# Yoshiki172/Deep-Learning-based-RGBA-Image-Compression-with-Masked-Window-based-Attention

Measured on NVIDIA B200. Metric: 768x512 RGBA images/s (AutoEncoderRGB_Journal encode + decode forward); masked-attn kernel % of roofline, higher is better.
Workload: dtype f32 (attention: fp16 hi+lo split operands, 3 tcgen05 passes, f32 accumulate = f32-faithful; 4x4 attention plain f32; GDN contraction bf16x3 split + f32 accumulate; convolutions fp16 hi+lo split operands, 3 tcgen05 passes, chunked f32 accumulation outside the tensor core = f32-faithful)

## Files before the change

deep-learning-based-rgba-image-compression-with-masked-window-based-attention_b200/_abi.py:

```python
from __future__ import annotations

import ctypes
import os
from ctypes import c_char_p, c_float, c_int, c_int32, c_int64, c_void_p, POINTER

import torch

_PKG_DIR = os.path.dirname(os.path.abspath(__file__))
LIB_PATH = os.path.join(_PKG_DIR, "libmwa_b200.so")

MWA_OK = 0
ALGO_AUTO, ALGO_SIMT, ALGO_TCGEN05 = 0, 1, 2
ABI_VERSION = 1

_SIGNATURES = {
    "mwa_b200_abi_version": (c_int, []),
    "mwa_b200_status_string": (c_char_p, [c_int]),
    "mwa_b200_last_cuda_error": (c_char_p, []),
    "gdn_param_bytes": (c_int64, [c_int]),
    "gdn_prepare": (c_int, [c_void_p, c_void_p, c_int, c_float, c_float, c_float, c_void_p, c_int64, c_void_p]),
    "gdn_forward": (c_int, [c_void_p, c_void_p, c_void_p, c_int64, c_int, c_int64, c_int, c_int, c_int, c_void_p]),
    "gdn_forward_planes": (c_int, [c_void_p, c_void_p, c_void_p, c_int, c_int, c_void_p, c_int64, c_int, c_int, c_int, c_int,
                                   c_void_p]),
    "gdn_backward_workspace_bytes": (c_int64, [c_int64, c_int, c_int64]),
# ... 3 lines not shown
    "gdn_bwd_square": (c_int, [c_void_p, c_void_p, c_int64, c_void_p]),
    "gdn_bwd_dn": (c_int, [c_void_p, c_void_p, c_void_p, c_void_p, c_void_p, c_int64, c_int, c_int64, c_int, c_int,
                           c_void_p]),
    "gdn_bwd_dx": (c_int, [c_void_p, c_void_p, c_void_p, c_void_p, c_int64, c_void_p]),
    "gdn_bwd_finalize": (c_int, [c_void_p, c_void_p, c_void_p, c_void_p, c_float, c_float, c_void_p, c_void_p,
                                 c_void_p, c_int64, c_int, c_int64, c_int, c_void_p]),
    "mwa_param_bytes": (c_int64, [c_int, c_int, c_int]),
    "mwa_prepare": (c_int, [c_void_p, c_void_p, c_void_p, c_void_p, c_void_p, c_int, c_int, c_int, c_float,
                            c_void_p, c_int64, c_void_p]),
    "mwa_debug_set_timing_buffer": (None, [c_void_p]),
    "mwa_workspace_bytes": (c_int64, [c_int, c_int, c_int, c_int]),
    "mwa_fast_path_needs_nchw": (c_int, [c_int, c_int, c_int]),
    "conv_image_bytes": (c_int64, [c_int, c_int, c_int, c_int, c_int]),
    "conv_split_bytes": (c_int64, [c_int, c_int, c_int, c_int]),
    "conv_prepare": (c_int, [c_void_p, c_int, c_int, c_int, c_int, c_int, c_void_p, c_int64, c_void_p]),
    "conv_forward": (c_int, [c_void_p, c_int64, c_void_p, c_void_p, c_void_p, c_int64, c_void_p, c_void_p, c_void_p, c_int,
                             c_int, c_int, c_int, c_int, c_int, c_int, c_int, c_int, c_void_p]),
    "gemm_tokens_forward": (c_int, [c_void_p, c_int64, c_int, c_void_p, c_void_p, c_int, c_void_p, c_void_p, c_void_p, c_void_p,
                                    c_void_p]),
    "conv_act_split": (c_int, [c_void_p, c_int64, c_int, c_int, c_int, c_int, c_int, c_void_p, c_void_p, c_int, c_int, c_void_p]),
    "conv_forward_ex": (c_int, [c_void_p, c_int64, c_void_p, c_void_p, c_int, c_void_p, c_void_p, c_void_p, c_int64,
                                c_void_p, c_int64, c_void_p, c_int64, c_void_p, c_void_p, c_int, c_int, c_int, c_void_p,
                                c_int, c_int, c_int, c_int, c_int, c_int, c_int, c_int, c_int, c_void_p, c_void_p]),
    "mwa_forward": (c_int, [c_void_p, c_void_p, c_void_p, c_void_p, c_int, c_int, c_int, c_int, c_int, c_int, c_int,
                            c_int, c_int, c_void_p, c_void_p, c_int64, c_void_p]),
    "window_attention_forward": (c_int, [c_void_p, c_void_p, c_void_p, c_void_p, c_int64, c_int, c_int, c_int, c_int,
                                         c_void_p]),
    "mwa_backward": (c_int, [c_void_p] * 12 + [c_int] * 8 + [c_void_p]),
    "window_attention_backward": (c_int, [c_void_p] * 10 + [c_int64, c_int, c_int, c_int, c_int, c_void_p]),
    "mwa_bwd_gather": (c_int, [c_void_p] * 6 + [c_int] * 7 + [c_void_p]),
    "mwa_bwd_core": (c_int, [c_void_p] * 8 + [c_int64] + [c_int] * 7 + [c_void_p]),
    "mwa_bwd_scatter": (c_int, [c_void_p] * 3 + [c_int] * 7 + [c_void_p]),
    "gate_residual_forward": (c_int, [c_void_p, c_void_p, c_void_p, c_void_p, c_int64, c_void_p]),
    "gate_residual_backward": (c_int, [c_void_p, c_void_p, c_void_p, c_void_p, c_void_p, c_int64, c_void_p]),
    "round_ste_forward": (c_int, [c_void_p, c_void_p, c_int64, c_int64, c_int64, c_int64, c_void_p]),
    "quantize_offset_forward": (c_int, [c_void_p, c_void_p, c_void_p, c_int64, c_int64, c_int64, c_int64, c_int64,
                                        c_int, c_int64, c_void_p]),
    "lrp_add_forward": (c_int, [c_void_p, c_void_p, c_void_p, c_int64, c_int64, c_int64, c_int64, c_int64, c_void_p]),
    "quantize_levels_forward": (c_int, [c_void_p, c_void_p, c_int64, c_float, c_void_p]),
    "alpha_pyramid_level_offset": (c_int64, [c_int, c_int, c_int, c_int]),
    "alpha_pyramid_forward": (c_int, [c_void_p, c_void_p, c_void_p, c_int, c_int, c_int, c_int, c_int, c_void_p]),
    "ms_ssim_level_forward": (c_int, [c_void_p, c_void_p, c_void_p, c_int, c_int, c_int, c_int, c_float, c_void_p, c_void_p,
                                      c_void_p]),
    "ms_ssim_pool_forward": (c_int, [c_void_p, c_void_p, c_void_p, c_int, c_int, c_int, c_int, c_void_p, c_void_p, c_void_p,
                                     c_void_p]),
    "rans_encode_with_indexes": (c_int64, [c_void_p, c_void_p, c_int64, c_void_p, c_int, c_void_p, c_void_p, c_int, c_void_p,
# ... 94 lines not shown
```

deep-learning-based-rgba-image-compression-with-masked-window-based-attention_b200/codec.py:

```python
from __future__ import annotations

import math

import numpy as np
import torch
import torch.nn as nn
import torch.nn.functional as F

from . import quant
from .layers.GDN import GDN
from .layers.Masked_Attention import Win_noShift_Attention, conv3x3
from .layers.conv import ACT_ADD2, ACT_LRP, ACT_QUANT, ACT_RELU, Conv2d, ConvStack, ConvTranspose2d, SplitAct
from .layers.SupplyMask import SupplyMaskToTransform, alpha_pyramid


def _conv(cin, cout, k, stride=1):
    return Conv2d(cin, cout, k, stride=stride, padding=k // 2)


def _deconv5(cin, cout):
    return ConvTranspose2d(cin, cout, 5, stride=2, padding=2, output_padding=1)


def _subpel(cin, cout, r=2):
    return nn.Sequential(Conv2d(cin, cout * r * r, 3, padding=1), nn.PixelShuffle(r))


class EnhancementBlock(nn.Module):

    def __init__(self, n=32):
        super().__init__()
        self.conv1 = Conv2d(n, n, 3, padding=1)
        self.relu = nn.ReLU(inplace=True)
        self.conv2 = Conv2d(n, n, 3, padding=1)

    def forward(self, x, **kw):
        if self.conv1.input_ps(x) is None:
            return self.conv2(self.conv1(x, act=ACT_RELU), residual=x)
        return self.conv2(self.conv1(x, act=ACT_RELU, emit_ps=1, want_dense=False),
                          residual=x.dense if isinstance(x, SplitAct) else x, **kw)


class DSE(nn.Module):

    def __init__(self, n=32):
        super().__init__()
        self.input_conv = Conv2d(3, n, 1)
        self.enh1, self.enh2, self.enh3 = EnhancementBlock(n), EnhancementBlock(n), EnhancementBlock(n)
        self.output_conv = Conv2d(n, 3, 1)

    def forward(self, x):
        if self.input_conv.input_ps(x) is None:
            first = self.input_conv(x)
            t = self.enh3(self.enh2(self.enh1(first)))
            return self.output_conv(t + first, residual=x)
        first = self.input_conv(x, emit_ps=1)
        t = self.enh2(self.enh1(first, emit_ps=1), emit_ps=1)
        h = self.enh3.conv1(t, act=ACT_RELU, emit_ps=1, want_dense=False)
        s = self.enh3.conv2(h, act=ACT_ADD2, residual=t.dense, aux=first.dense, emit_ps=1, want_dense=False)
        return self.output_conv(s, residual=x)


def _gdn_into(gdn, x, consumer):
    ps = consumer.input_ps(x) if torch.is_tensor(x) and x.dim() == 4 and x.shape[1] == consumer.in_channels else None
    return gdn.request_planes(ps)(x) if ps else gdn(x)


def _attention_into(attention, x, mask, consumer):
    ps = consumer.input_ps(x) if torch.is_tensor(x) and x.dim() == 4 and x.shape[1] == consumer.in_channels else None
    if ps and attention.conv_a[0].conv[0].input_ps(x) is not None:
        return attention.request_planes(ps)(x, mask)
    return attention(x, mask)


class Analysis_transform(nn.Module):

    def __init__(self, N=192, M=320):
        super().__init__()
        self.x1 = _conv(3, N, 5, 2)
        self.gdn1 = GDN(N)
        self.x2 = _conv(N, N, 5, 2)
        self.gdn2 = GDN(N)
        self.attention1 = Win_noShift_Attention(dim=N, num_heads=8, window_size=8, shift_size=4)
        self.x3 = _conv(N, N, 5, 2)
        self.gdn3 = GDN(N)
        self.x4 = Conv2d(N, M, 1)
        self.attention2 = Win_noShift_Attention(dim=M, num_heads=8, window_size=4, shift_size=2)

    def forward(self, input, mask, me1, me2, me3, me4):
        y = _gdn_into(self.gdn1, self.x1(input), self.x2)
        y = self.gdn2(self.x2(y))
        y = _attention_into(self.attention1, y, me2, self.x3)
        y = _gdn_into(self.gdn3, self.x3(y), self.x4)
        return self.attention2(self.x4(y), me3)


class Synthesis_transform(nn.Module):

    def __init__(self, N=196, M=320):
        super().__init__()
        self.attention1 = Win_noShift_Attention(dim=M, num_heads=8, window_size=4, shift_size=2)
        self.x1 = Conv2d(M, N, 1)
        self.igdn1 = GDN(N, inverse=True)
        self.x2 = _deconv5(N, N)
        self.igdn2 = GDN(N, inverse=True)
        self.attention2 = Win_noShift_Attention(N, num_heads=8, window_size=8, shift_size=4)
        self.x3 = _deconv5(N, N)
        self.igdn3 = GDN(N, inverse=True)
        self.x4 = _deconv5(N, 3)
        self.dse = DSE(32)

    def forward(self, input, reconmask, md1, md2, md3, md4):
        y = _attention_into(self.attention1, input, md3, self.x1)
        y = _gdn_into(self.igdn1, self.x1(y), self.x2)
        y = self.igdn2(self.x2(y))
        y = _attention_into(self.attention2, y, md2, self.x3)
        y = _gdn_into(self.igdn3, self.x3(y), self.x4)
        return self.dse(self.x4(y))


class EntropyBottleneck(nn.Module):

    def __init__(self, channels, filters=(3, 3, 3, 3), init_scale=10.0):
        super().__init__()
        self.channels = channels
        f = (1,) + tuple(filters) + (1,)
        scale = init_scale ** (1.0 / (len(filters) + 1))
        for i in range(len(filters) + 1):
            init = math.log(math.expm1(1.0 / scale / f[i + 1]))
            self.register_parameter(f"_matrix{i:d}", nn.Parameter(torch.full((channels, f[i + 1], f[i]), init)))
            self.register_parameter(f"_bias{i:d}", nn.Parameter(torch.rand(channels, f[i + 1], 1) - 0.5))
            if i < len(filters):
                self.register_parameter(f"_factor{i:d}", nn.Parameter(torch.zeros(channels, f[i + 1], 1)))
        self.nlayers = len(filters) + 1
        self.quantiles = nn.Parameter(torch.tensor([-init_scale, 0.0, init_scale]).repeat(channels, 1, 1))

    def _get_medians(self):
        return self.quantiles[:, :, 1:2].detach().reshape(1, -1, 1, 1)

    def _logits_cumulative(self, v):
        for i in range(self.nlayers):
# ... 364 lines not shown
```

deep-learning-based-rgba-image-compression-with-masked-window-based-attention_b200/csrc/conv_tc.cu:

```cuda
#include <cstring>
#include <cuda.h>
#include "common.cuh"
#include "params.cuh"
#include "status.cuh"

namespace b200 {
namespace {

__host__ __device__ constexpr int conv_colparts(int nbmax) { return nbmax <= 64 ? 2 : 4; }
__host__ __device__ constexpr int conv_threads(int nbmax) { return (3 + 4 * conv_colparts(nbmax)) * 32; }
constexpr int kMaxTaps = 25, kMaxClasses = 4, kMaxGroups = 4;
constexpr int kTileH = 16, kTileW = 8;
enum { kActNone = 0, kActGelu = 1, kActRelu = 2, kActQuant = 3, kActLrp = 4, kActGate = 5, kActAdd2 = 6 };

struct ConvIo {
    const float* bias;
    const float* residual;
    float* out;
    int64_t out_bs;
    const float* aux;
    int64_t aux_bs;
    float* out2;
    int64_t out2_bs;
    uint16_t* sp_hi;
    uint16_t* sp_lo;
    int sp_ps, sp_cstride, sp_coff, sp_cvalid;
    const float* in_scale;
    int out_cl;
};

struct ConvTap {
    int16_t row;
    int16_t slab;
};
struct ConvGroup {
    int8_t plane, ntaps;
    int16_t first;
};
struct ConvPlan {
    int B, Cin, Cout, Npad, nblocks, nb;
    int KB;
    int GH, GW;
    int Ho, Wo, os;
    int ncls;
    int ntaps[kMaxClasses], ngroups[kMaxClasses];
    int8_t qy[kMaxClasses], qx[kMaxClasses];
    ConvGroup groups[kMaxClasses][kMaxGroups];
    ConvTap taps[kMaxClasses][kMaxTaps];
    int th, tw, tw_log2;
    int hy, hx, oy0, ox0;
    int a_half;
    int act;
    int merged;
    int nslabs;
    int sa, sb;
    int bparts;
    int resident;
    int dual;
    int nbuf_log2, bstride;
    int ncat;
    int b_region;
    int chunk;
    int nchunks[kMaxClasses];
    int tiles_y, tiles_x;
};

__device__ __forceinline__ uint64_t umma_desc_k_sw128_sbo(uint32_t smem_addr, uint32_t sbo_bytes) {
    uint64_t d = 0;
    d |= static_cast<uint64_t>((smem_addr & 0x3FFFFu) >> 4);
    d |= static_cast<uint64_t>(1) << 16;
    d |= static_cast<uint64_t>(sbo_bytes >> 4) << 32;
    d |= static_cast<uint64_t>(1) << 46;
    d |= static_cast<uint64_t>(2) << 61;
    return d;
}

__device__ __forceinline__ void tma_load_5d(void* dst_smem, const void* map, int c0, int c1, int c2, int c3, int c4, uint64_t* bar) {
    asm volatile(
        "cp.async.bulk.tensor.5d.shared::cluster.global.tile.mbarrier::complete_tx::bytes [%0], [%1, {%2,%3,%4,%5,%6}], [%7];" ::"r"(
            smem_u32(dst_smem)),
        "l"(map), "r"(c0), "r"(c1), "r"(c2), "r"(c3), "r"(c4), "r"(smem_u32(bar))
        : "memory");
}

__device__ __forceinline__ uint16_t conv_f16_bits(float v) { return __half_as_ushort(__float2half_rn(v)); }

__global__ void __launch_bounds__(256)
// ... 220 lines not shown
        } else {
            y[u] = v + rv[u];
        }
        if (!FULL && u >= nvalid) y[u] = 0.f;
    }
    if (dst != nullptr) {
#pragma unroll
        for (int u = 0; u < 8; ++u)
            if (FULL || u < nvalid) dst[u * ohw] = y[u];
    }
    if (sph != nullptr) {
        uint32_t hi[4], lo[4];
#pragma unroll
        for (int u = 0; u < 4; ++u) {
            hi[u] = pack_f16x2(y[2 * u], y[2 * u + 1]);
            const float2 hf = __half22float2(*reinterpret_cast<const __half2*>(&hi[u]));
            lo[u] = pack_f16x2(y[2 * u] - hf.x, y[2 * u + 1] - hf.y);
        }
        *reinterpret_cast<uint4*>(sph) = make_uint4(hi[0], hi[1], hi[2], hi[3]);
        *reinterpret_cast<uint4*>(spl) = make_uint4(lo[0], lo[1], lo[2], lo[3]);
    }
}

template <int NBMAX, bool kCL = false, bool kSingle = false>
__global__ void __launch_bounds__(conv_threads(NBMAX), 1)
conv_tc_kernel(const __grid_constant__ CUtensorMap map_hi, const __grid_constant__ CUtensorMap map_lo,
               const uint8_t* __restrict__ image, const float* __restrict__ inv_scale, const __grid_constant__ ConvIo io,
               const __grid_constant__ ConvPlan P) {
    extern __shared__ __align__(1024) uint8_t smem[];
    __shared__ uint64_t bars[2 * 4 + 2 * 8 + 2 * 4];
    __shared__ uint32_t tmem_slot;
    __shared__ uint2 s_tap[kMaxClasses * kMaxTaps + 1];
    const uint32_t sb = smem_u32(smem);
    const int warp = threadIdx.x >> 5, lane = threadIdx.x & 31;
    const int SA = P.sa, SB = P.sb;
    uint64_t* a_full = bars;
    uint64_t* a_empty = bars + 4;
    uint64_t* b_full = bars + 8;
    uint64_t* b_empty = bars + 16;
    uint64_t* part_full = bars + 24;
    uint64_t* part_empty = bars + 28;
    const uint32_t nbl = uint32_t(P.nbuf_log2), nbm = (1u << nbl) - 1u, bstride = uint32_t(P.bstride);
    const uint32_t b_bytes = uint32_t(P.nb) * 128u;
    const uint32_t b_entry = P.bparts == 2 ? b_bytes : 2u * b_bytes;
    const uint32_t a_slot = 2u * uint32_t(P.a_half);
    const uint32_t b_base = uint32_t(SA) * a_slot;
    if (threadIdx.x == 0) {
        if (sb & 1023u) __trap();
        for (int i = 0; i < SA; ++i) {
            mbar_init(a_full + i, 1);
            mbar_init(a_empty + i, 1);
        }
        for (int i = 0; i < SB; ++i) {
            mbar_init(b_full + i, 1);
            mbar_init(b_empty + i, 1);
        }
        for (int i = 0; i < 4; ++i) {
            mbar_init(part_full + i, 1);
            mbar_init(part_empty + i, 4 * conv_colparts(NBMAX) * 32);
        }
        fence_mbar_init();
    }
    if (warp == 1) tmem_alloc<512>(&tmem_slot);
    float* s_scale = reinterpret_cast<float*>(smem + b_base + P.b_region);
    float* s_bias = s_scale + P.Npad;
    for (int i = threadIdx.x; i < P.Npad; i += conv_threads(NBMAX)) {
        s_scale[i] = inv_scale[i] * (io.in_scale ? 1.f / __ldg(io.in_scale) : 1.f);
        const int co = P.merged ? (i & 7) : i;
        s_bias[i] = (io.bias != nullptr && co < P.Cout) ? io.bias[co] : 0.f;
    }
    for (int i = threadIdx.x; i < kMaxClasses * kMaxTaps; i += conv_threads(NBMAX)) {
        const ConvTap tp = P.taps[i / kMaxTaps][i % kMaxTaps];
        s_tap[i] = make_uint2(uint32_t(tp.row) * 8u, uint32_t(tp.slab * P.KB * 2) * ((uint32_t(P.nb) * 128u) >> 4));
    }
    tc_fence_before_sync();
    __syncthreads();
    tc_fence_after_sync();
    const uint32_t tm = tmem_slot;

    const int tiles_img = P.tiles_y * P.tiles_x;
    const int ntiles = P.B * tiles_img * P.ncls * P.nblocks;
    struct TileIt {
        int nblk, tx, ty, cls, b;
        int d_nblk, d_tx, d_ty, d_cls, d_b;
        __device__ __forceinline__ void init(int t, int step, const ConvPlan& P) {
            auto split = [&](int v, int& nb_, int& tx_, int& ty_, int& cl_, int& b_) {
                nb_ = v % P.nblocks; v /= P.nblocks;
                tx_ = v % P.tiles_x; v /= P.tiles_x;
                ty_ = v % P.tiles_y; v /= P.tiles_y;
                cl_ = v % P.ncls;
                b_ = v / P.ncls;
            };
// ... 275 lines not shown
                                    for (int j = 0; j < 8; ++j) acc[c0 + 8 + j] += __uint_as_float(v1[j]);
                                }
                            }
                        }
                    }
                    if (ch < nchunks - 1) {
                        tc_fence_before_sync();
                        mbar_arrive(part_empty + buf);
                    } else {
#pragma unroll
                        for (int c0 = 0; c0 < NBQ; c0 += 8) {
                            if (c0 < ncols) {
                                uint32_t v[8];
#pragma unroll
                                for (int j = 0; j < 8; ++j) v[j] = __float_as_uint(acc[c0 + j]);
                                tmem_st_x8(tm + lane_addr + buf * bstride + col0 + c0, v);
                            }
                        }
                        tmem_wait_st();
                    }
                }
            }
            if (nchunks == 1) ++c;
            float* dst = io.out ? (kCL ? io.out + pix * io.out_bs + cbase : io.out + b * io.out_bs + cbase * ohw + pix) : nullptr;
            float* dst2 = io.out2 ? io.out2 + b * io.out2_bs + cbase * ohw + pix : nullptr;
            int64_t spo = 0;
            if (io.sp_hi != nullptr) {
                const int sh = io.sp_ps - 1;
                const int hp = P.Ho >> sh, wp = P.Wo >> sh;
                const int plane = ((oy & sh) << sh) + (ox & sh);
                spo = (((int64_t(b) << (2 * sh)) + plane) * hp + (oy >> sh)) * wp + (ox >> sh);
                spo = spo * io.sp_cstride + io.sp_coff + cbase;
            }
            const int act = P.act;
            const int64_t estride = kCL ? 1 : ohw;
#pragma unroll 1
            for (int j0 = 0; j0 < ncols; j0 += 8) {
                uint32_t tv[8];
                tmem_ld_x8(tm + lane_addr + buf * bstride + col0 + j0, tv);
                if (NBMAX <= 64 && P.ncat && nchunks == 1) {
                    uint32_t t2[8];
                    tmem_ld_x8(tm + lane_addr + buf * bstride + P.nb + col0 + j0, t2);
                    tmem_wait_ld();
#pragma unroll
                    for (int u = 0; u < 8; ++u) tv[u] = __float_as_uint(__uint_as_float(tv[u]) + __uint_as_float(t2[u]));
                }
// ... 175 lines not shown
    P.bparts = P.nb > 96 ? 2 : 1;
    if (P.nblocks == 1 && image <= budget) {
        P.resident = 1; P.bparts = 1; P.sb = 1; P.b_region = int(image);
    } else {
        const int entry = P.nb * 128 * (P.bparts == 2 ? 1 : 2);
        P.sb = budget / entry;
        if (P.sb > 8) P.sb = 8;
        if (P.sb < 2) return MWA_ERR_UNSUPPORTED;
        P.b_region = P.sb * entry;
    }
    P.dual = P.resident && P.ncls == 1 && P.ngroups[0] == 1 && P.KB == 1 && P.nchunks[0] == 1 && P.ntaps[0] > 1;
    P.ncat = P.nb <= 64 ? 1 : 0;
    P.nbuf_log2 = (P.nb <= 128 && !P.dual) ? 2 : 1;
    P.bstride = P.nbuf_log2 == 2 ? 128 : 256;
    if (P.dual) {
        const int room = 224 * 1024 - 2 * P.Npad * 4 - P.b_region;
        P.sa = room / (2 * P.a_half);
        if (P.sa > 4) P.sa = 4;
        if (P.sa < 2) P.sa = 2;
    }
    return MWA_OK;
}

int conv_smem_bytes(const ConvPlan& P) { return P.sa * 2 * P.a_half + P.b_region + 2 * P.Npad * 4 + 1024; }

}
}

using namespace b200;

extern "C" {

int64_t conv_image_bytes(int kind, int Cin, int Cout, int k, int stride) {
    ConvPlan P;
    if (Cin <= 0 || Cout <= 0 || build_plan(P, kind, 1, Cin, Cout, 16, 16, k, stride, 0) != MWA_OK) return MWA_ERR_UNSUPPORTED;
    return int64_t(P.nslabs) * P.KB * 2 * P.Npad * 128 + int64_t(P.Npad) * 4;
}

int64_t conv_split_bytes(int B, int Cin, int H, int W) {
    const int64_t Cpad = (Cin + 7) / 8 * 8;
    return int64_t(B) * H * W * Cpad * 2;
}

int conv_prepare(const float* w, int kind, int Cin, int Cout, int k, int stride, void* image, int64_t image_bytes, void* stream) {
    if (!w || !image) return MWA_ERR_INVALID;
    const int wflip = kind == 2;
    if (wflip) {
// ... 10 lines not shown
    float* inv_scale = reinterpret_cast<float*>(img + int64_t(P.nslabs) * P.KB * 2 * P.Npad * 128);
    const int wmode = P.merged ? 3 : wflip ? 2 : kind;
    conv_prepare_kernel<<<P.Npad, 256, 0, static_cast<cudaStream_t>(stream)>>>(w, Cin, Cout, k, wmode, P.Npad, P.KB, P.nslabs,
                                                                              inv_scale, img);
    return check_launch("conv_prepare");
}

int conv_act_split(const float* x, int64_t x_batch_stride, int B, int C, int H, int W, int ps, void* out_hi, void* out_lo,
                   int out_cstride, int out_coff, void* stream) {
    if (!x || !out_hi || !out_lo || B < 0 || C <= 0 || H <= 0 || W <= 0 || (ps != 1 && ps != 2)) return MWA_ERR_INVALID;
    const int Cpad = (C + 7) / 8 * 8;
    if (out_cstride % 8 != 0 || out_coff % 8 != 0 || out_coff < 0 || out_coff + Cpad > out_cstride || H % ps || W % ps)
        return MWA_ERR_INVALID;
    if (!aligned16(out_hi) || !aligned16(out_lo)) return MWA_ERR_ALIGNMENT;
    if (B == 0) return MWA_OK;
    return launch_act_split(x, x_batch_stride, B, C, out_cstride, H, W, ps, static_cast<uint16_t*>(out_hi) + out_coff,
                            static_cast<uint16_t*>(out_lo) + out_coff, static_cast<cudaStream_t>(stream));
}

static int conv_forward_impl(const float* x, int64_t x_batch_stride, void* in_hi, void* in_lo, int in_cstride,
                    const float* bias, const float* residual, float* out, int64_t out_batch_stride, const float* aux,
                    int64_t aux_batch_stride, float* out2, int64_t out2_batch_stride, void* out_hi, void* out_lo,
                    int out_ps, int out_cstride, int out_coff, const void* image, int kind, int B, int Cin, int Cout, int H,
                    int W, int k, int stride, int act, const float* in_scale, void* stream, int out_cl) {
    if (!image || !in_hi || !in_lo || (!out && !out_hi)) return MWA_ERR_INVALID;
    if (B < 0 || Cin <= 0 || Cout <= 0 || H <= 0 || W <= 0 || act < 0 || act > kActAdd2) return MWA_ERR_INVALID;
    if (act >= kActQuant && !aux) return MWA_ERR_INVALID;
    if ((out_hi != nullptr) != (out_lo != nullptr)) return MWA_ERR_INVALID;
    if (B == 0) return MWA_OK;
    ConvPlan P;
    int rc = build_plan(P, kind, B, Cin, Cout, H, W, k, stride, act);
    if (rc != MWA_OK) return rc;
    if (!aligned16(in_hi) || !aligned16(in_lo) || !aligned16(image)) return MWA_ERR_ALIGNMENT;
    if (P.merged && (out_hi != nullptr || act >= kActQuant)) return MWA_ERR_UNSUPPORTED;
    if (int64_t(B) * Cout * P.Ho * P.Wo >= (int64_t(1) << 31)) return MWA_ERR_UNSUPPORTED;
    cudaStream_t st = static_cast<cudaStream_t>(stream);
    const int ps = (kind == 0 && stride == 2) ? 2 : 1;
    int cstride = in_cstride;
    if (x != nullptr) {
        cstride = (Cin + 7) / 8 * 8;
        rc = launch_act_split(x, x_batch_stride, B, Cin, cstride, H, W, ps, static_cast<uint16_t*>(in_hi),
                              static_cast<uint16_t*>(in_lo), st, in_scale);
        if (rc != MWA_OK) return rc;
    } else if (cstride < Cin || cstride % 8 != 0) {
        return MWA_ERR_INVALID;
    }
    ConvIo io;
    memset(&io, 0, sizeof(io));
    io.bias = bias; io.residual = residual; io.out = out; io.out_bs = out_batch_stride;
    io.aux = aux; io.aux_bs = aux_batch_stride; io.out2 = out2; io.out2_bs = out2_batch_stride;
    io.in_scale = in_scale;
    io.out_cl = out_cl;
    if (out_hi != nullptr) {
        if (!aligned16(out_hi) || !aligned16(out_lo)) return MWA_ERR_ALIGNMENT;
        if ((out_ps != 1 && out_ps != 2) || out_cstride % 8 != 0 || out_coff % 8 != 0 || out_coff < 0 ||
            out_coff + (Cout + 7) / 8 * 8 > out_cstride || P.Ho % out_ps != 0 || P.Wo % out_ps != 0)
            return MWA_ERR_INVALID;
        io.sp_hi = static_cast<uint16_t*>(out_hi); io.sp_lo = static_cast<uint16_t*>(out_lo);
        io.sp_ps = out_ps; io.sp_cstride = out_cstride; io.sp_coff = out_coff; io.sp_cvalid = (Cout + 7) / 8 * 8;
    }
    CUtensorMap mh, ml;
    memset(&mh, 0, sizeof(mh));
    memset(&ml, 0, sizeof(ml));
    rc = conv_plane_map(in_hi, B, ps * ps, H / ps, W / ps, Cin, cstride, P.hx, P.hy, &mh);
    if (rc != MWA_OK) return rc;
    rc = conv_plane_map(in_lo, B, ps * ps, H / ps, W / ps, Cin, cstride, P.hx, P.hy, &ml);
    if (rc != MWA_OK) return rc;
    const int smem = conv_smem_bytes(P);
    const int ntiles = B * P.tiles_y * P.tiles_x * P.ncls * P.nblocks;
    const int grid = ntiles < kNumSMs ? ntiles : kNumSMs;
    const uint8_t* img = static_cast<const uint8_t*>(image);
    const float* inv_scale = reinterpret_cast<const float*>(img + int64_t(P.nslabs) * P.KB * 2 * P.Npad * 128);
#define CONV_LAUNCH_K(NB, SINGLE)                                                                                              \
    do {                                                                                                                       \
        MWA_TRY_CUDA(cudaFuncSetAttribute(conv_tc_kernel<NB, false, SINGLE>, cudaFuncAttributeMaxDynamicSharedMemorySize, smem), \
                     "conv_forward(attr)");                                                                                    \
        conv_tc_kernel<NB, false, SINGLE><<<grid, conv_threads(NB), smem, st>>>(mh, ml, img, inv_scale, io, P);                \
    } while (0)
#define CONV_LAUNCH(NB)                                                                                                        \
    do {                                                                                                                       \
        if (NB >= 128 && single) CONV_LAUNCH_K(NB, (NB >= 128));                                                               \
        else CONV_LAUNCH_K(NB, false);                                                                                         \
    } while (0)
    bool single = true;
    for (int c = 0; c < P.ncls; ++c) single = single && P.nchunks[c] == 1;
    if (out_cl) {
        MWA_TRY_CUDA(cudaFuncSetAttribute(conv_tc_kernel<192, true>, cudaFuncAttributeMaxDynamicSharedMemorySize, smem),
                     "gemm_tokens_forward(attr)");
        conv_tc_kernel<192, true><<<grid, conv_threads(192), smem, st>>>(mh, ml, img, inv_scale, io, P);
        return check_launch("gemm_tokens_forward");
    }
    if (P.nb <= 32) CONV_LAUNCH(32);
    else if (P.nb <= 64) CONV_LAUNCH(64);
    else if (P.nb <= 128) CONV_LAUNCH(128);
    else CONV_LAUNCH(192);
#undef CONV_LAUNCH
#undef CONV_LAUNCH_K
    return check_launch("conv_forward");
}

int conv_forward_ex(const float* x, int64_t x_batch_stride, void* in_hi, void* in_lo, int in_cstride,
                    const float* bias, const float* residual, float* out, int64_t out_batch_stride, const float* aux,
                    int64_t aux_batch_stride, float* out2, int64_t out2_batch_stride, void* out_hi, void* out_lo,
                    int out_ps, int out_cstride, int out_coff, const void* image, int kind, int B, int Cin, int Cout, int H,
                    int W, int k, int stride, int act, const float* in_scale, void* stream) {
    return conv_forward_impl(x, x_batch_stride, in_hi, in_lo, in_cstride, bias, residual, out, out_batch_stride, aux,
                             aux_batch_stride, out2, out2_batch_stride, out_hi, out_lo, out_ps, out_cstride, out_coff, image,
                             kind, B, Cin, Cout, H, W, k, stride, act, in_scale, stream, 0);
}

int gemm_tokens_forward(const float* x, int64_t T, int Cin, const float* bias, float* out, int Cout, const void* image,
                        void* split_hi, void* split_lo, const float* in_scale, void* stream) {
    if (!x || !out || !image || !split_hi || !split_lo || T < 0 || Cin <= 0 || Cout <= 0) return MWA_ERR_INVALID;
    if (T == 0) return MWA_OK;
    if (T % 32 != 0 || Cout % 8 != 0 || T / 32 > 2000000) return MWA_ERR_UNSUPPORTED;
    if (!aligned16(x) || !aligned16(out) || !aligned16(split_hi) || !aligned16(split_lo)) return MWA_ERR_ALIGNMENT;
    const int cstride = (Cin + 7) / 8 * 8;
    cudaStream_t st = static_cast<cudaStream_t>(stream);
    const int64_t items = T * ((Cin + 7) / 8);
    int64_t blocks = (items + 255) / 256;
    if (blocks > kNumSMs * 16) blocks = kNumSMs * 16;
    conv_split_cl_kernel<<<unsigned(blocks), 256, 0, st>>>(x, T, Cin, cstride, static_cast<uint16_t*>(split_hi),
                                                          static_cast<uint16_t*>(split_lo), in_scale);
    int rc = check_launch("gemm_tokens_forward(split)");
    if (rc != MWA_OK) return rc;
    return conv_forward_impl(nullptr, 0, split_hi, split_lo, cstride, bias, nullptr, out, Cout, nullptr, 0, nullptr, 0, nullptr,
                             nullptr, 0, 0, 0, image, 0, 1, Cin, Cout, int(T / 32), 32, 1, 1, kActNone, in_scale, stream, 1);
}

int conv_forward(const float* x, int64_t x_batch_stride, const float* bias, const float* residual, float* out,
                 int64_t out_batch_stride, const void* image, void* split_hi, void* split_lo, int kind, int B, int Cin,
// ... 8 lines not shown
```

deep-learning-based-rgba-image-compression-with-masked-window-based-attention_b200/layers/conv.py:

```python
from __future__ import annotations

import torch
import torch.nn as nn
import torch.nn.functional as F

from .. import _abi

ACT_NONE, ACT_GELU, ACT_RELU, ACT_QUANT, ACT_LRP, ACT_GATE, ACT_ADD2 = 0, 1, 2, 3, 4, 5, 6


def _act_of(m):
    if isinstance(m, nn.GELU) and getattr(m, "approximate", "none") == "none":
        return ACT_GELU
    if isinstance(m, nn.ReLU):
        return ACT_RELU
    return None


def _apply_act(y, act):
    return F.gelu(y) if act == ACT_GELU else F.relu(y) if act == ACT_RELU else y


class SplitAct:

# ... 67 lines not shown


GEMM_TOKENS_MIN_FLOP = 2e9
USE_KERNEL = True


def _fast_ok(x, *tensors):
    if not USE_KERNEL:
        return False
    if isinstance(x, SplitAct):
        return True
    if not (x.is_cuda and x.dtype == torch.float32 and x.dim() == 4 and x.numel() > 0):
        return False
    if torch.is_grad_enabled() and (x.requires_grad or any(t is not None and t.requires_grad for t in tensors)):
        return False
    return _dense_nchw(x)


def _run(x, bias, image, kind, k, stride, act, residual, cout, ho, wo, emit_ps=0, want_dense=True, aux=None, out=None,
         out2=None, emit_into=None, in_scale=None):
    lib = _abi.load()
    B, cin, H, W = x.shape
    dev = x.device
    if isinstance(x, SplitAct):
        need_ps = 2 if (kind == 0 and stride == 2) else 1
        if x.ps != need_ps:
            raise RuntimeError(f"conv: split input has ps {x.ps}, this convolution needs {need_ps}")
        xp, xbs, in_hi, in_lo, in_cs = None, 0, x.hi, x.lo, x.cstride
    else:
        nsplit = int(lib.conv_split_bytes(B, cin, H, W))
        scratch = torch.empty(2, nsplit, dtype=torch.uint8, device=dev)
        xp, xbs, in_hi, in_lo, in_cs = x.data_ptr(), x.stride(0), scratch[0], scratch[1], 0
    if out is None and want_dense:
        out = torch.empty(B, cout, ho, wo, device=dev, dtype=torch.float32)
    if out is not None and (tuple(out.shape) != (B, cout, ho, wo) or not _dense_nchw(out)):
        raise RuntimeError(f"conv: bad output tensor {tuple(out.shape)} / {out.stride()}")
    if residual is not None:
        if tuple(residual.shape) != (B, cout, ho, wo):
            raise RuntimeError(f"conv: residual shape {tuple(residual.shape)} != output shape {(B, cout, ho, wo)}")
        residual = residual.contiguous()
    for name, t in (("aux", aux), ("out2", out2)):
        if t is not None and (tuple(t.shape) != (B, cout, ho, wo) or not _dense_nchw(t)):
            raise RuntimeError(f"conv: bad {name} tensor {tuple(t.shape)} / {t.stride()}")
    sp, coff = None, 0
    if emit_into is not None:
        sp, coff = emit_into
    elif emit_ps:
        sp = SplitAct.empty(B, cout, ho, wo, emit_ps, dev)
    b = None if bias is None else bias.detach().contiguous()
    with torch.cuda.device(dev):
        _abi.check(lib.conv_forward_ex(
            xp, xbs, in_hi.data_ptr(), in_lo.data_ptr(), in_cs, _abi.ptr(b), _abi.ptr(residual), _abi.ptr(out),
            0 if out is None else out.stride(0), _abi.ptr(aux), 0 if aux is None else aux.stride(0), _abi.ptr(out2),
            0 if out2 is None else out2.stride(0), None if sp is None else sp.hi.data_ptr(),
            None if sp is None else sp.lo.data_ptr(), 0 if sp is None else sp.ps, 0 if sp is None else sp.cstride, coff,
            image.data_ptr(), kind, B, cin, cout, H, W, k, stride, act, _abi.ptr(in_scale), _abi.stream_handle()),
            "conv_forward_ex")
    _abi.count_launches(1 if xp is None else 2)
    if sp is None:
        return out
    if emit_into is None:
        sp.dense = out
        return sp
    return out


def _dense_nchw(t):
    C, H, W = t.shape[1:]
    return t.stride(3) == 1 and t.stride(2) == W and t.stride(1) == H * W and t.stride(0) >= C * H * W


class _ShapeOnly:

    is_cuda, dtype, requires_grad = True, torch.float32, False

    def __init__(self, shape, device):
        self.shape, self.device = tuple(shape), device

    def dim(self):
        return len(self.shape)

    def numel(self):
        n = 1
        for v in self.shape:
            n *= v
        return n

    def stride(self, i):
        st = [1] * len(self.shape)
# ... 246 lines not shown
```

include/mwa_b200.h:

```cpp
#ifndef MWA_B200_H_
#define MWA_B200_H_

#include <stdint.h>

#if defined(__GNUC__)
#define MWA_API __attribute__((visibility("default")))
#else
#define MWA_API
#endif

#ifdef __cplusplus
extern "C" {
#endif

#define MWA_B200_ABI_VERSION 1

enum {
    MWA_OK = 0,
    MWA_ERR_INVALID = -1,
    MWA_ERR_UNSUPPORTED = -2,
    MWA_ERR_ALIGNMENT = -3,
    MWA_ERR_WORKSPACE = -4,
    MWA_ERR_CUDA = -5
};
// ... 75 lines not shown
MWA_API int alpha_pyramid_forward(const float* alpha, float* recon, float* levels, int B, int H, int W, int nlevels,
                                  int quant_levels, void* stream);

MWA_API int mask_constraint_forward(const float* mask, float* out, int B, int H, int W, int quant_levels, void* stream);

MWA_API int64_t conv_image_bytes(int kind, int Cin, int Cout, int k, int stride);
MWA_API int64_t conv_split_bytes(int B, int Cin, int H, int W);
MWA_API int conv_prepare(const float* w, int kind, int Cin, int Cout, int k, int stride, void* image, int64_t image_bytes,
                         void* stream);
MWA_API int conv_forward(const float* x, int64_t x_batch_stride, const float* bias, const float* residual, float* out,
                         int64_t out_batch_stride, const void* image, void* split_hi, void* split_lo, int kind, int B,
                         int Cin, int Cout, int H, int W, int k, int stride, int act, void* stream);

MWA_API int gemm_tokens_forward(const float* x, int64_t T, int Cin, const float* bias, float* out, int Cout, const void* image,
                                void* split_hi, void* split_lo, const float* in_scale, void* stream);
MWA_API int conv_act_split(const float* x, int64_t x_batch_stride, int B, int C, int H, int W, int ps, void* out_hi,
                           void* out_lo, int out_cstride, int out_coff, void* stream);
MWA_API int conv_forward_ex(const float* x, int64_t x_batch_stride, void* in_hi, void* in_lo, int in_cstride,
                            const float* bias, const float* residual, float* out, int64_t out_batch_stride,
                            const float* aux, int64_t aux_batch_stride, float* out2, int64_t out2_batch_stride,
                            void* out_hi, void* out_lo, int out_ps, int out_cstride, int out_coff, const void* image,
                            int kind, int B, int Cin, int Cout, int H, int W, int k, int stride, int act,
                            const float* in_scale, void* stream);

MWA_API int ms_ssim_level_forward(const float* X, const float* Y, const float* mask, int B, int C, int H, int W,
                                  float data_range, float* sums, float* counts, void* stream);
MWA_API int ms_ssim_pool_forward(const float* X, const float* Y, const float* mask, int B, int C, int H, int W, float* Xo,
                                 float* Yo, float* Mo, void* stream);

MWA_API int64_t rans_encode_with_indexes(const int32_t* symbols, const int32_t* indexes, int64_t n, const int32_t* cdfs,
                                         int cdf_stride, const int32_t* cdf_sizes, const int32_t* offsets, int ncdf,
                                         uint8_t* out, int64_t out_capacity);
MWA_API int rans_decode_with_indexes(const uint8_t* stream, int64_t nbytes, int64_t* state, const int32_t* indexes, int64_t n,
                                     const int32_t* cdfs, int cdf_stride, const int32_t* cdf_sizes, const int32_t* offsets,
                                     int ncdf, int32_t* symbols_out);

#define MWA_RANS_LANES_MAGIC 0x4C41574Du
#define MWA_RANS_LANES_VERSION 1u
MWA_API int rans_lanes_encode(const int32_t* symbols, const int32_t* indexes, int n_streams, int64_t n, int lanes,
                              const int32_t* cdfs, int cdf_stride, const int32_t* cdf_sizes, const int32_t* offsets,
                              int ncdf, uint32_t* slots, int64_t slot_words, int32_t* lane_words, void* stream);
MWA_API int rans_lanes_pack(const uint32_t* slots, int64_t slot_words, const int32_t* lane_words, int n_streams, int lanes,
                            int64_t* lane_dst, int64_t* stream_bytes, uint32_t* out, int64_t out_words, void* stream);
MWA_API int rans_lanes_decode(const uint32_t* data, int64_t data_words, int64_t* lane_state, int total_lanes,
                              const int32_t* stream_lanes, int n_streams, const int32_t* indexes, int64_t n,
                              int64_t position, const int32_t* cdfs, int cdf_stride, const int32_t* cdf_sizes,
// ... 12 lines not shown
```

Before: 385.3.

## Fuse DSE 1x1 input/output convs into neighbouring tcgen05 conv epilogues

Adds two fused variants of the tensor-core conv kernel. The final 5x5 stride-2 deconvolution to RGB now also computes the DSE input 1x1 conv (3->32) in its epilogue and writes both dense and fp16 hi/lo split copies. The last enhancement 3x3 conv applies the ADD2 residual, then the 3-channel 1x1 output conv and the image residual in its epilogue, using a shared-memory exchange between the two column halves. This removes separate launches and the round trips of the 32-channel full-resolution intermediates through global memory, at the cost of extra epilogue work and shared memory.

```diff
diff --git a/deep-learning-based-rgba-image-compression-with-masked-window-based-attention_b200/_abi.py b/deep-learning-based-rgba-image-compression-with-masked-window-based-attention_b200/_abi.py
--- a/deep-learning-based-rgba-image-compression-with-masked-window-based-attention_b200/_abi.py
+++ b/deep-learning-based-rgba-image-compression-with-masked-window-based-attention_b200/_abi.py
@@ -49,6 +49,10 @@
     "conv_forward_ex": (c_int, [c_void_p, c_int64, c_void_p, c_void_p, c_int, c_void_p, c_void_p, c_void_p, c_int64,
                                 c_void_p, c_int64, c_void_p, c_int64, c_void_p, c_void_p, c_int, c_int, c_int, c_void_p,
                                 c_int, c_int, c_int, c_int, c_int, c_int, c_int, c_int, c_int, c_void_p, c_void_p]),
+    "deconv_dse_in_forward": (c_int, [c_void_p, c_int64, c_void_p, c_void_p, c_int, c_void_p, c_void_p, c_void_p, c_int, c_int,
+                                      c_int, c_int, c_void_p, c_void_p, c_void_p, c_void_p, c_void_p, c_int, c_void_p]),
+    "conv_dse_out_forward": (c_int, [c_void_p, c_void_p, c_int, c_void_p, c_void_p, c_void_p, c_void_p, c_int, c_int, c_int,
+                                     c_void_p, c_void_p, c_void_p, c_void_p, c_void_p]),
     "mwa_forward": (c_int, [c_void_p, c_void_p, c_void_p, c_void_p, c_int, c_int, c_int, c_int, c_int, c_int, c_int,
                             c_int, c_int, c_void_p, c_void_p, c_int64, c_void_p]),
     "window_attention_forward": (c_int, [c_void_p, c_void_p, c_void_p, c_void_p, c_int64, c_int, c_int, c_int, c_int,
diff --git a/deep-learning-based-rgba-image-compression-with-masked-window-based-attention_b200/codec.py b/deep-learning-based-rgba-image-compression-with-masked-window-based-attention_b200/codec.py
--- a/deep-learning-based-rgba-image-compression-with-masked-window-based-attention_b200/codec.py
+++ b/deep-learning-based-rgba-image-compression-with-masked-window-based-attention_b200/codec.py
@@ -10,8 +10,12 @@
 from . import quant
 from .layers.GDN import GDN
 from .layers.Masked_Attention import Win_noShift_Attention, conv3x3
-from .layers.conv import ACT_ADD2, ACT_LRP, ACT_QUANT, ACT_RELU, Conv2d, ConvStack, ConvTranspose2d, SplitAct
+from .layers.conv import (ACT_ADD2, ACT_LRP, ACT_QUANT, ACT_RELU, Conv2d, ConvStack, ConvTranspose2d, SplitAct, _ShapeOnly,
+                          conv_dse_out, deconv_dse_in)
 from .layers.SupplyMask import SupplyMaskToTransform, alpha_pyramid
+
+
+FUSED_DSE = True
 
 
 def _conv(cin, cout, k, stride=1):
@@ -49,14 +53,25 @@
         self.enh1, self.enh2, self.enh3 = EnhancementBlock(n), EnhancementBlock(n), EnhancementBlock(n)
         self.output_conv = Conv2d(n, 3, 1)
 
-    def forward(self, x):
-        if self.input_conv.input_ps(x) is None:
+    def fusable(self, deconv, y):
+        if not (FUSED_DSE and deconv.out_channels == 3 and self.input_conv.out_channels == 32):
+            return False
+        if deconv.input_ps(y) is None:
+            return False
+        B, _, H, W = y.shape
+        return self.input_conv.input_ps(_ShapeOnly((B, 3, 2 * H, 2 * W), y.device)) is not None
+
+    def forward(self, x, first=None):
+        if first is None and self.input_conv.input_ps(x) is None:
             first = self.input_conv(x)
             t = self.enh3(self.enh2(self.enh1(first)))
             return self.output_conv(t + first, residual=x)
-        first = self.input_conv(x, emit_ps=1)
+        if first is None:
+            first = self.input_conv(x, emit_ps=1)
         t = self.enh2(self.enh1(first, emit_ps=1), emit_ps=1)
         h = self.enh3.conv1(t, act=ACT_RELU, emit_ps=1, want_dense=False)
+        if FUSED_DSE:
+            return conv_dse_out(self.enh3.conv2, h, t.dense, first.dense, self.output_conv, x)
         s = self.enh3.conv2(h, act=ACT_ADD2, residual=t.dense, aux=first.dense, emit_ps=1, want_dense=False)
         return self.output_conv(s, residual=x)
 
@@ -71,6 +86,12 @@
     if ps and attention.conv_a[0].conv[0].input_ps(x) is not None:
         return attention.request_planes(ps)(x, mask)
     return attention(x, mask)
+
+
+def _deconv_dse(deconv, y, dse):
+    if dse.fusable(deconv, y):
+        return dse(*deconv_dse_in(deconv, y, dse.input_conv))
+    return dse(deconv(y))
 
 
 class Analysis_transform(nn.Module):
@@ -116,7 +137,7 @@
         y = self.igdn2(self.x2(y))
         y = _attention_into(self.attention2, y, md2, self.x3)
         y = _gdn_into(self.igdn3, self.x3(y), self.x4)
-        return self.dse(self.x4(y))
+        return _deconv_dse(self.x4, y, self.dse)
 
 
 class EntropyBottleneck(nn.Module):
diff --git a/deep-learning-based-rgba-image-compression-with-masked-window-based-attention_b200/csrc/conv_tc.cu b/deep-learning-based-rgba-image-compression-with-masked-window-based-attention_b200/csrc/conv_tc.cu
--- a/deep-learning-based-rgba-image-compression-with-masked-window-based-attention_b200/csrc/conv_tc.cu
+++ b/deep-learning-based-rgba-image-compression-with-masked-window-based-attention_b200/csrc/conv_tc.cu
@@ -12,6 +12,9 @@
 constexpr int kMaxTaps = 25, kMaxClasses = 4, kMaxGroups = 4;
 constexpr int kTileH = 16, kTileW = 8;
 enum { kActNone = 0, kActGelu = 1, kActRelu = 2, kActQuant = 3, kActLrp = 4, kActGate = 5, kActAdd2 = 6 };
+enum { kFuseNone = 0, kFuseDseIn = 1, kFuseDseOut = 2 };
+constexpr int kDseWidth = 32, kDseRgb = 3;
+constexpr int kFuseSmem = (kDseWidth + 1) * 16 + 2 * kDseRgb * 128 * 4;
 
 struct ConvIo {
     const float* bias;
@@ -27,6 +30,10 @@
     int sp_ps, sp_cstride, sp_coff, sp_cvalid;
     const float* in_scale;
     int out_cl;
+    const float* fw;
+    const float* fb;
+    const float* fres;
+    float* fout;
 };
 
 struct ConvTap {
@@ -63,6 +70,7 @@
     int chunk;
     int nchunks[kMaxClasses];
     int tiles_y, tiles_x;
+    int fuse;
 };
 
 __device__ __forceinline__ uint64_t umma_desc_k_sw128_sbo(uint32_t smem_addr, uint32_t sbo_bytes) {
@@ -329,7 +337,19 @@
     }
 }
 
-template <int NBMAX, bool kCL = false, bool kSingle = false>
+__device__ __forceinline__ void store_split8(const float (&y)[8], uint16_t* sph, uint16_t* spl) {
+    uint32_t hi[4], lo[4];
+#pragma unroll
+    for (int u = 0; u < 4; ++u) {
+        hi[u] = pack_f16x2(y[2 * u], y[2 * u + 1]);
+        const float2 hf = __half22float2(*reinterpret_cast<const __half2*>(&hi[u]));
+        lo[u] = pack_f16x2(y[2 * u] - hf.x, y[2 * u + 1] - hf.y);
+    }
+    *reinterpret_cast<uint4*>(sph) = make_uint4(hi[0], hi[1], hi[2], hi[3]);
+    *reinterpret_cast<uint4*>(spl) = make_uint4(lo[0], lo[1], lo[2], lo[3]);
+}
+
+template <int NBMAX, bool kCL = false, bool kSingle = false, int kFuse = kFuseNone>
 __global__ void __launch_bounds__(conv_threads(NBMAX), 1)
 conv_tc_kernel(const __grid_constant__ CUtensorMap map_hi, const __grid_constant__ CUtensorMap map_lo,
                const uint8_t* __restrict__ image, const float* __restrict__ inv_scale, const __grid_constant__ ConvIo io,
@@ -375,6 +395,16 @@
         s_scale[i] = inv_scale[i] * (io.in_scale ? 1.f / __ldg(io.in_scale) : 1.f);
         const int co = P.merged ? (i & 7) : i;
         s_bias[i] = (io.bias != nullptr && co < P.Cout) ? io.bias[co] : 0.f;
+    }
+    float4* s_fuse = reinterpret_cast<float4*>(s_bias + P.Npad);
+    float* s_xch = reinterpret_cast<float*>(s_fuse + kDseWidth + 1);
+    if constexpr (kFuse == kFuseDseIn) {
+        for (int i = threadIdx.x; i < kDseWidth; i += conv_threads(NBMAX))
+            s_fuse[i] = make_float4(io.fw[i * kDseRgb], io.fw[i * kDseRgb + 1], io.fw[i * kDseRgb + 2], io.fb[i]);
+    } else if constexpr (kFuse == kFuseDseOut) {
+        for (int i = threadIdx.x; i <= kDseWidth; i += conv_threads(NBMAX))
+            s_fuse[i] = i < kDseWidth ? make_float4(io.fw[i], io.fw[kDseWidth + i], io.fw[2 * kDseWidth + i], 0.f)
+                                      : make_float4(io.fb[0], io.fb[1], io.fb[2], 0.f);
     }
     for (int i = threadIdx.x; i < kMaxClasses * kMaxTaps; i += conv_threads(NBMAX)) {
         const ConvTap tp = P.taps[i / kMaxTaps][i % kMaxTaps];
@@ -696,6 +726,86 @@
                 }
             }
             if (nchunks == 1) ++c;
+            if constexpr (kFuse != kFuseNone) {
+                auto granule = [&](int j0, uint32_t (&tv)[8]) {
+                    tmem_ld_x8(tm + lane_addr + buf * bstride + col0 + j0, tv);
+                    if (P.ncat && nchunks == 1) {
+                        uint32_t t2[8];
+                        tmem_ld_x8(tm + lane_addr + buf * bstride + P.nb + col0 + j0, t2);
+                        tmem_wait_ld();
+#pragma unroll
+                        for (int u = 0; u < 8; ++u) tv[u] = __float_as_uint(__uint_as_float(tv[u]) + __uint_as_float(t2[u]));
+                    }
+                    tmem_wait_ld();
+                };
+                if constexpr (kFuse == kFuseDseIn) {
+                    uint32_t tv[2][8];
+                    granule(0, tv[0]);
+                    granule(8, tv[1]);
+                    if (inb) {
+                        const int64_t p0 = int64_t(oy + cq) * P.Wo + ox;
+                        float xv[2][kDseRgb];
+#pragma unroll
+                        for (int p = 0; p < 2; ++p)
+#pragma unroll
+                            for (int u = 0; u < kDseRgb; ++u) {
+                                const int cc = col0 + 8 * p + u;
+                                xv[p][u] = fmaf(__uint_as_float(tv[p][u]), s_scale[cc], s_bias[cc]);
+                                io.out[b * io.out_bs + u * ohw + p0 + p] = xv[p][u];
+                            }
+                        float* fo = io.fout + int64_t(b) * kDseWidth * ohw + p0;
+                        const int64_t sp0 = (int64_t(b) * ohw + p0) * io.sp_cstride + io.sp_coff;
+#pragma unroll
+                        for (int g = 0; g < kDseWidth; g += 8) {
+                            float f[2][8];
+#pragma unroll
+                            for (int u = 0; u < 8; ++u) {
+                                const float4 w = s_fuse[g + u];
+#pragma unroll
+                                for (int p = 0; p < 2; ++p) f[p][u] = fmaf(w.z, xv[p][2], fmaf(w.y, xv[p][1], fmaf(w.x, xv[p][0], w.w)));
+                                *reinterpret_cast<float2*>(fo + (g + u) * ohw) = make_float2(f[0][u], f[1][u]);
+                            }
+                            store_split8(f[0], io.sp_hi + sp0 + g, io.sp_lo + sp0 + g);
+                            store_split8(f[1], io.sp_hi + sp0 + io.sp_cstride + g, io.sp_lo + sp0 + io.sp_cstride + g);
+                        }
+                    }
+                } else {
+                    float o[kDseRgb] = {0.f, 0.f, 0.f};
+#pragma unroll
+                    for (int j0 = 0; j0 < 16; j0 += 8) {
+                        uint32_t tv[8];
+                        granule(j0, tv);
+                        if (inb) {
+#pragma unroll
+                            for (int u = 0; u < 8; ++u) {
+                                const int cc = col0 + j0 + u;
+                                const float v = fmaf(__uint_as_float(tv[u]), s_scale[cc], s_bias[cc]);
+                                const float sv = (v + __ldg(res + (j0 + u) * ohw)) + aux[(j0 + u) * ohw];
+                                const float4 w = s_fuse[cc];
+                                o[0] = fmaf(w.x, sv, o[0]);
+                                o[1] = fmaf(w.y, sv, o[1]);
+                                o[2] = fmaf(w.z, sv, o[2]);
+                            }
+                        }
+                    }
+                    float* xch = s_xch + (c & 1) * (kDseRgb * 128);
+                    if (cq == 1) {
+#pragma unroll
+                        for (int k = 0; k < kDseRgb; ++k) xch[k * 128 + r] = o[k];
+                    }
+                    asm volatile("bar.sync %0, 64;" ::"r"(1 + q) : "memory");
+                    if (cq == 0 && inb) {
+                        const float4 bo = s_fuse[kDseWidth];
+                        const int64_t xo = int64_t(b) * kDseRgb * ohw + pix;
+                        io.fout[xo] = ((o[0] + xch[r]) + bo.x) + __ldg(io.fres + xo);
+                        io.fout[xo + ohw] = ((o[1] + xch[128 + r]) + bo.y) + __ldg(io.fres + xo + ohw);
+                        io.fout[xo + 2 * ohw] = ((o[2] + xch[256 + r]) + bo.z) + __ldg(io.fres + xo + 2 * ohw);
+                    }
+                }
+                tc_fence_before_sync();
+                mbar_arrive(part_empty + buf);
+                continue;
+            }
             float* dst = io.out ? (kCL ? io.out + pix * io.out_bs + cbase : io.out + b * io.out_bs + cbase * ohw + pix) : nullptr;
             float* dst2 = io.out2 ? io.out2 + b * io.out2_bs + cbase * ohw + pix : nullptr;
             int64_t spo = 0;
@@ -917,7 +1027,9 @@
     return MWA_OK;
 }
 
-int conv_smem_bytes(const ConvPlan& P) { return P.sa * 2 * P.a_half + P.b_region + 2 * P.Npad * 4 + 1024; }
+int conv_smem_bytes(const ConvPlan& P) {
+    return P.sa * 2 * P.a_half + P.b_region + 2 * P.Npad * 4 + (P.fuse ? kFuseSmem : 0) + 1024;
+}
 
 }
 }
@@ -974,8 +1086,10 @@
                     const float* bias, const float* residual, float* out, int64_t out_batch_stride, const float* aux,
                     int64_t aux_batch_stride, float* out2, int64_t out2_batch_stride, void* out_hi, void* out_lo,
                     int out_ps, int out_cstride, int out_coff, const void* image, int kind, int B, int Cin, int Cout, int H,
-                    int W, int k, int stride, int act, const float* in_scale, void* stream, int out_cl) {
-    if (!image || !in_hi || !in_lo || (!out && !out_hi)) return MWA_ERR_INVALID;
+                    int W, int k, int stride, int act, const float* in_scale, void* stream, int out_cl,
+                    int fuse = kFuseNone, const float* fw = nullptr, const float* fb = nullptr, const float* fres = nullptr,
+                    float* fout = nullptr) {
+    if (!image || !in_hi || !in_lo || (!out && !out_hi && !fout)) return MWA_ERR_INVALID;
     if (B < 0 || Cin <= 0 || Cout <= 0 || H <= 0 || W <= 0 || act < 0 || act > kActAdd2) return MWA_ERR_INVALID;
     if (act >= kActQuant && !aux) return MWA_ERR_INVALID;
     if ((out_hi != nullptr) != (out_lo != nullptr)) return MWA_ERR_INVALID;
@@ -984,7 +1098,21 @@
     int rc = build_plan(P, kind, B, Cin, Cout, H, W, k, stride, act);
     if (rc != MWA_OK) return rc;
     if (!aligned16(in_hi) || !aligned16(in_lo) || !aligned16(image)) return MWA_ERR_ALIGNMENT;
-    if (P.merged && (out_hi != nullptr || act >= kActQuant)) return MWA_ERR_UNSUPPORTED;
+    if (P.merged && fuse == kFuseNone && (out_hi != nullptr || act >= kActQuant)) return MWA_ERR_UNSUPPORTED;
+    if (fuse != kFuseNone) {
+        if (!fw || !fb || !fout || !aligned16(fout)) return MWA_ERR_INVALID;
+        if (fuse == kFuseDseIn) {
+            if (!P.merged || Cout != kDseRgb || act != kActNone || residual || !out || !out_hi || out_ps != 1 ||
+                out_coff + kDseWidth > out_cstride)
+                return MWA_ERR_INVALID;
+        } else {
+            if (kind != 0 || k != 3 || stride != 1 || Cin != kDseWidth || Cout != kDseWidth || act != kActAdd2 || !residual ||
+                out || out_hi || !fres)
+                return MWA_ERR_INVALID;
+        }
+        if (P.nb != 32 || P.nblocks != 1) return MWA_ERR_UNSUPPORTED;
+        P.fuse = fuse;
+    }
     if (int64_t(B) * Cout * P.Ho * P.Wo >= (int64_t(1) << 31)) return MWA_ERR_UNSUPPORTED;
     cudaStream_t st = static_cast<cudaStream_t>(stream);
     const int ps = (kind == 0 && stride == 2) ? 2 : 1;
@@ -1003,6 +1131,7 @@
     io.aux = aux; io.aux_bs = aux_batch_stride; io.out2 = out2; io.out2_bs = out2_batch_stride;
     io.in_scale = in_scale;
     io.out_cl = out_cl;
+    io.fw = fw; io.fb = fb; io.fres = fres; io.fout = fout;
     if (out_hi != nullptr) {
         if (!aligned16(out_hi) || !aligned16(out_lo)) return MWA_ERR_ALIGNMENT;
         if ((out_ps != 1 && out_ps != 2) || out_cstride % 8 != 0 || out_coff % 8 != 0 || out_coff < 0 ||
@@ -1019,6 +1148,7 @@
     rc = conv_plane_map(in_lo, B, ps * ps, H / ps, W / ps, Cin, cstride, P.hx, P.hy, &ml);
     if (rc != MWA_OK) return rc;
     const int smem = conv_smem_bytes(P);
+    if (smem > 227 * 1024) return MWA_ERR_UNSUPPORTED;
     const int ntiles = B * P.tiles_y * P.tiles_x * P.ncls * P.nblocks;
     const int grid = ntiles < kNumSMs ? ntiles : kNumSMs;
     const uint8_t* img = static_cast<const uint8_t*>(image);
@@ -1042,6 +1172,18 @@
         conv_tc_kernel<192, true><<<grid, conv_threads(192), smem, st>>>(mh, ml, img, inv_scale, io, P);
         return check_launch("gemm_tokens_forward");
     }
+    if (fuse != kFuseNone) {
+        if (fuse == kFuseDseIn) {
+            MWA_TRY_CUDA(cudaFuncSetAttribute(conv_tc_kernel<32, false, false, kFuseDseIn>,
+                                              cudaFuncAttributeMaxDynamicSharedMemorySize, smem), "deconv_dse_in_forward(attr)");
+            conv_tc_kernel<32, false, false, kFuseDseIn><<<grid, conv_threads(32), smem, st>>>(mh, ml, img, inv_scale, io, P);
+        } else {
+            MWA_TRY_CUDA(cudaFuncSetAttribute(conv_tc_kernel<32, false, false, kFuseDseOut>,
+                                              cudaFuncAttributeMaxDynamicSharedMemorySize, smem), "conv_dse_out_forward(attr)");
+            conv_tc_kernel<32, false, false, kFuseDseOut><<<grid, conv_threads(32), smem, st>>>(mh, ml, img, inv_scale, io, P);
+        }
+        return check_launch(fuse == kFuseDseIn ? "deconv_dse_in_forward" : "conv_dse_out_forward");
+    }
     if (P.nb <= 32) CONV_LAUNCH(32);
     else if (P.nb <= 64) CONV_LAUNCH(64);
     else if (P.nb <= 128) CONV_LAUNCH(128);
@@ -1059,6 +1201,24 @@
     return conv_forward_impl(x, x_batch_stride, in_hi, in_lo, in_cstride, bias, residual, out, out_batch_stride, aux,
                              aux_batch_stride, out2, out2_batch_stride, out_hi, out_lo, out_ps, out_cstride, out_coff, image,
                              kind, B, Cin, Cout, H, W, k, stride, act, in_scale, stream, 0);
+}
+
+int deconv_dse_in_forward(const float* x, int64_t x_batch_stride, void* in_hi, void* in_lo, int in_cstride, const float* bias,
+                          float* out, const void* image, int B, int Cin, int H, int W, const float* w_in, const float* b_in,
+                          float* first, void* first_hi, void* first_lo, int first_cstride, void* stream) {
+    if (!out || !aligned16(out)) return MWA_ERR_INVALID;
+    return conv_forward_impl(x, x_batch_stride, in_hi, in_lo, in_cstride, bias, nullptr, out, int64_t(kDseRgb) * 4 * H * W,
+                             nullptr, 0, nullptr, 0, first_hi, first_lo, 1, first_cstride, 0, image, 1, B, Cin, kDseRgb, H, W,
+                             5, 2, kActNone, nullptr, stream, 0, kFuseDseIn, w_in, b_in, nullptr, first);
+}
+
+int conv_dse_out_forward(void* in_hi, void* in_lo, int in_cstride, const float* bias, const float* t, const float* first,
+                         const void* image, int B, int H, int W, const float* w_out, const float* b_out, const float* x,
+                         float* x_hat, void* stream) {
+    if (!t || !first) return MWA_ERR_INVALID;
+    return conv_forward_impl(nullptr, 0, in_hi, in_lo, in_cstride, bias, t, nullptr, 0, first, int64_t(kDseWidth) * H * W,
+                             nullptr, 0, nullptr, nullptr, 0, 0, 0, image, 0, B, kDseWidth, kDseWidth, H, W, 3, 1, kActAdd2,
+                             nullptr, stream, 0, kFuseDseOut, w_out, b_out, x, x_hat);
 }
 
 int gemm_tokens_forward(const float* x, int64_t T, int Cin, const float* bias, float* out, int Cout, const void* image,
diff --git a/deep-learning-based-rgba-image-compression-with-masked-window-based-attention_b200/layers/conv.py b/deep-learning-based-rgba-image-compression-with-masked-window-based-attention_b200/layers/conv.py
--- a/deep-learning-based-rgba-image-compression-with-masked-window-based-attention_b200/layers/conv.py
+++ b/deep-learning-based-rgba-image-compression-with-masked-window-based-attention_b200/layers/conv.py
@@ -113,15 +113,7 @@
     lib = _abi.load()
     B, cin, H, W = x.shape
     dev = x.device
-    if isinstance(x, SplitAct):
-        need_ps = 2 if (kind == 0 and stride == 2) else 1
-        if x.ps != need_ps:
-            raise RuntimeError(f"conv: split input has ps {x.ps}, this convolution needs {need_ps}")
-        xp, xbs, in_hi, in_lo, in_cs = None, 0, x.hi, x.lo, x.cstride
-    else:
-        nsplit = int(lib.conv_split_bytes(B, cin, H, W))
-        scratch = torch.empty(2, nsplit, dtype=torch.uint8, device=dev)
-        xp, xbs, in_hi, in_lo, in_cs = x.data_ptr(), x.stride(0), scratch[0], scratch[1], 0
+    xp, xbs, in_hi, in_lo, in_cs = _input_operands(lib, x, 2 if (kind == 0 and stride == 2) else 1)
     if out is None and want_dense:
         out = torch.empty(B, cout, ho, wo, device=dev, dtype=torch.float32)
     if out is not None and (tuple(out.shape) != (B, cout, ho, wo) or not _dense_nchw(out)):
@@ -156,6 +148,59 @@
     return out
 
 
+def _input_operands(lib, x, need_ps):
+    if isinstance(x, SplitAct):
+        if x.ps != need_ps:
+            raise RuntimeError(f"conv: split input has ps {x.ps}, this convolution needs {need_ps}")
+        return None, 0, x.hi, x.lo, x.cstride
+    B, cin, H, W = x.shape
+    scratch = torch.empty(2, int(lib.conv_split_bytes(B, cin, H, W)), dtype=torch.uint8, device=x.device)
+    return x.data_ptr(), x.stride(0), scratch[0], scratch[1], 0
+
+
+def _bias_of(m):
+    return m.bias.detach().contiguous() if m.bias is not None else torch.zeros(m.out_channels, device=m.weight.device)
+
+
+def deconv_dse_in(deconv, x, conv_in):
+    lib = _abi.load()
+    B, cin, H, W = x.shape
+    dev = x.device
+    img = deconv._img.get(deconv.weight, 1, 5, 2)
+    xp, xbs, in_hi, in_lo, in_cs = _input_operands(lib, x, 1)
+    out = torch.empty(B, 3, 2 * H, 2 * W, device=dev, dtype=torch.float32)
+    n = conv_in.out_channels
+    first = SplitAct.empty(B, n, 2 * H, 2 * W, 1, dev)
+    first.dense = torch.empty(B, n, 2 * H, 2 * W, device=dev, dtype=torch.float32)
+    w_in = conv_in.weight.detach().reshape(n, 3).contiguous()
+    b_in = _bias_of(conv_in)
+    b = None if deconv.bias is None else deconv.bias.detach().contiguous()
+    with torch.cuda.device(dev):
+        _abi.check(lib.deconv_dse_in_forward(
+            xp, xbs, in_hi.data_ptr(), in_lo.data_ptr(), in_cs, _abi.ptr(b), out.data_ptr(), img.data_ptr(), B, cin, H, W,
+            w_in.data_ptr(), b_in.data_ptr(), first.dense.data_ptr(), first.hi.data_ptr(), first.lo.data_ptr(), first.cstride,
+            _abi.stream_handle()), "deconv_dse_in_forward")
+    _abi.count_launches(1 if xp is None else 2)
+    return out, first
+
+
+def conv_dse_out(conv, h, t, first, conv_out, x):
+    lib = _abi.load()
+    B, n, H, W = t.shape
+    img = conv._img.get(conv.weight, 0, 3, 1)
+    t, first, x = t.contiguous(), first.contiguous(), x.contiguous()
+    x_hat = torch.empty_like(x)
+    w_out = conv_out.weight.detach().reshape(3, n).contiguous()
+    b_out = _bias_of(conv_out)
+    b = None if conv.bias is None else conv.bias.detach().contiguous()
+    with torch.cuda.device(t.device):
+        _abi.check(lib.conv_dse_out_forward(
+            h.hi.data_ptr(), h.lo.data_ptr(), h.cstride, _abi.ptr(b), t.data_ptr(), first.data_ptr(), img.data_ptr(), B, H, W,
+            w_out.data_ptr(), b_out.data_ptr(), x.data_ptr(), x_hat.data_ptr(), _abi.stream_handle()), "conv_dse_out_forward")
+    _abi.count_launches(1)
+    return x_hat
+
+
 def _dense_nchw(t):
     C, H, W = t.shape[1:]
     return t.stride(3) == 1 and t.stride(2) == W and t.stride(1) == H * W and t.stride(0) >= C * H * W
diff --git a/include/mwa_b200.h b/include/mwa_b200.h
--- a/include/mwa_b200.h
+++ b/include/mwa_b200.h
@@ -121,6 +121,13 @@
                             void* out_hi, void* out_lo, int out_ps, int out_cstride, int out_coff, const void* image,
                             int kind, int B, int Cin, int Cout, int H, int W, int k, int stride, int act,
                             const float* in_scale, void* stream);
+MWA_API int deconv_dse_in_forward(const float* x, int64_t x_batch_stride, void* in_hi, void* in_lo, int in_cstride,
+                                  const float* bias, float* out, const void* image, int B, int Cin, int H, int W,
+                                  const float* w_in, const float* b_in, float* first, void* first_hi, void* first_lo,
+                                  int first_cstride, void* stream);
+MWA_API int conv_dse_out_forward(void* in_hi, void* in_lo, int in_cstride, const float* bias, const float* t,
+                                 const float* first, const void* image, int B, int H, int W, const float* w_out,
+                                 const float* b_out, const float* x, float* x_hat, void* stream);
 
 MWA_API int ms_ssim_level_forward(const float* X, const float* Y, const float* mask, int B, int C, int H, int W,
                                   float data_range, float* sums, float* counts, void* stream);
```

After: 393.2 (median of 6 runs). 1.02x the previous value.
